# hridaybavle/semantic_slam

Measured on AMD Instinct MI355X. Metric: graph-optimize LM iters/sec (5k poses, 1k landmarks), higher is better.
Workload: dtype f64

## Files before the change

### include/sslam.h

```cpp
#ifndef SSLAM_H
#define SSLAM_H

#include <stdint.h>

#ifdef __cplusplus
extern "C" {
#endif

#define SSLAM_OK 0
#define SSLAM_ERR_INVALID (-1)
#define SSLAM_ERR_NO_DEVICE (-2)
#define SSLAM_ERR_HIP (-3)
#define SSLAM_ERR_NUMERIC (-4)
#define SSLAM_ERR_TOO_FEW_EDGES (-5)
#define SSLAM_ERR_UNSUPPORTED (-6)
#define SSLAM_ERR_IO (-7)

const char* sslam_last_error(void);
int sslam_device_count(void);
void* sslam_pinned_alloc(size_t bytes);
void sslam_pinned_free(void* p);

typedef struct sslam_graph sslam_graph;

// ... 68 lines not shown
sslam_batch* sslam_batch_create(sslam_graph* const* graphs, int n);
sslam_batch* sslam_batch_create_streams(sslam_graph* const* graphs, int n, int n_streams);
void sslam_batch_destroy(sslam_batch* b);
int sslam_batch_upload(sslam_batch* b);
int sslam_batch_download(sslam_batch* b);
int sslam_batch_optimize(sslam_batch* b, int max_iters, sslam_opt_stats* out );
int sslam_batch_marginals(sslam_batch* b, const int32_t* req, int n, double* out_blocks);
int sslam_comm_unique_id(char id_out[128]);
int sslam_batch_comm_init(sslam_batch* b, const char id_in[128], int rank, int world);
int sslam_batch_set_edge_shard(sslam_batch* b, int rank, int world);
int64_t sslam_batch_linearize_hb(sslam_batch* b, double* h_and_b, int64_t capacity);
int sslam_batch_time_linearize(sslam_batch* b, int repeats, double* ms_per_build);
int sslam_batch_time_solver(sslam_batch* b, int repeats, double* factor_ms, double* solve_ms);
int64_t sslam_batch_linearize_bytes(const sslam_batch* b);
int sslam_batch_info(sslam_batch* b, const char* key, double* value);
int sslam_batch_set_profiling(sslam_batch* b, int enable);
int sslam_batch_kernel_time(sslam_batch* b, const char* name, double* total_ms, int64_t* launches);

typedef struct sslam_seg sslam_seg;

typedef struct sslam_seg_params {
  double num_point_seg;
  double norm_point_thres;
  double planar_area;
  float max_depth_change_factor;
  float normal_smoothing_size;
  float angular_threshold;
  float distance_threshold;
  float maximum_curvature;
  int min_contour_points;
// ... 154 lines not shown
```

### semantic_slam_amd/_lib.py

```python
from __future__ import annotations

import ctypes as C
import os
import subprocess

_PKG = os.path.dirname(os.path.abspath(__file__))
_LIB = None


def library_path() -> str:
    return os.path.join(_PKG, "libsslam_hip.so")


def build_library(force: bool = False) -> str:
    args = ["make", "-C", os.path.join(_PKG, "csrc"), "-s"]
    if force:
        args.append("-B")
    subprocess.check_call(args)
    return library_path()


class OptStats(C.Structure):
    _fields_ = [("iterations", C.c_int), ("trials", C.c_int), ("status", C.c_int), ("host_plan_us", C.c_int),
                ("chi2_before", C.c_double), ("chi2_after", C.c_double), ("lambda_", C.c_double),
# ... 56 lines not shown
        "sslam_batch_create": (vp, [C.POINTER(vp), ci]),
        "sslam_batch_create_streams": (vp, [C.POINTER(vp), ci, ci]),
        "sslam_batch_destroy": (None, [vp]),
        "sslam_batch_upload": (ci, [vp]),
        "sslam_batch_download": (ci, [vp]),
        "sslam_batch_optimize": (ci, [vp, ci, C.POINTER(OptStats)]),
        "sslam_batch_marginals": (ci, [vp, C.POINTER(C.c_int32), ci, dp]),
        "sslam_comm_unique_id": (ci, [C.c_char_p]),
        "sslam_batch_comm_init": (ci, [vp, C.c_char_p, ci, ci]),
        "sslam_batch_set_edge_shard": (ci, [vp, ci, ci]),
        "sslam_batch_linearize_hb": (i64, [vp, dp, i64]),
        "sslam_batch_time_linearize": (ci, [vp, ci, dp]),
        "sslam_batch_time_solver": (ci, [vp, ci, dp, dp]),
        "sslam_batch_linearize_bytes": (i64, [vp]),
        "sslam_batch_info": (ci, [vp, C.c_char_p, dp]),
        "sslam_batch_set_profiling": (ci, [vp, ci]),
        "sslam_batch_kernel_time": (ci, [vp, C.c_char_p, dp, C.POINTER(i64)]),
    }
    for name, (res, args) in sig.items():
        fn = getattr(lib, name)
        fn.restype = res
        fn.argtypes = args
    _LIB = lib
    return lib
```

### semantic_slam_amd/csrc/chol_plan.hpp

```cpp
#pragma once
#include <algorithm>
#include <array>
#include <cstdint>
#include <cstdio>
#include <cstdlib>
#include <cstring>
#include <functional>
#include <map>
#include <queue>
#include <string>
#include <unordered_map>
#include <utility>
#include <vector>

namespace sslam {
#ifdef SSLAM_PLAN_TIMERS
#include <chrono>
#define SSLAM_PT_INIT auto pt_ = std::chrono::steady_clock::now();
#define SSLAM_PT(name) { auto n_ = std::chrono::steady_clock::now(); fprintf(stderr, "[plan-timer] %-14s %.3f ms\n", name, std::chrono::duration<double, std::milli>(n_ - pt_).count()); pt_ = n_; }
#else
#define SSLAM_PT_INIT
#define SSLAM_PT(name)
#endif

// ... 61 lines not shown
};
struct CholOpts {
  int cap_leaf = -1;
  int cap_tail = 4608;
  int max_blocks = 224;
  int tail_width = -1;
  int mid_width = -1;
  int cap_mid = 1800;
  int nt_mid = 128;
  int nt_ftail = 256;
  int pcap_mid = 16;
  int nt_bleaf = 0, nt_bmid = 0, nt_btail = 0;
  int nt_leaf = -1, nt_tail = 512;
  int min_chunk = 4;
  int split_min = 4096;
  int pcap_leaf = 4, pcap_tail = 32;
  int group_cap = -1;
  int group_blocks = 1024;
  int ustage = -1;
  int order = 1;
  double order_mul = -1;
  int order_add = -1;
  int order_bits_max = 2048;
  bool dump = false;
  int front = -1;
  int flow = 1;
  void from_env() {
    {
      static bool warned = false;
      if (!warned) {
// ... 10 lines not shown
    std::string str(e);
    size_t pos = 0;
    while (pos < str.size()) {
      size_t end = str.find(',', pos);
      if (end == std::string::npos) end = str.size();
      const std::string kv = str.substr(pos, end - pos);
      pos = end + 1;
      const size_t eq = kv.find('=');
      if (eq == std::string::npos) continue;
      const std::string k = kv.substr(0, eq), v = kv.substr(eq + 1);
      const int iv = atoi(v.c_str());
      if (k == "cap_leaf") cap_leaf = iv; else if (k == "cap_mid") cap_mid = iv; else if (k == "cap_tail") cap_tail = iv;
      else if (k == "max_blocks") max_blocks = iv; else if (k == "tail_width") tail_width = iv; else if (k == "mid_width") mid_width = iv;
      else if (k == "nt_leaf") { nt_leaf = iv; nt_leaf_set = true; } else if (k == "nt_mid") nt_mid = iv; else if (k == "nt_ftail") nt_ftail = iv; else if (k == "nt_bleaf") nt_bleaf = iv; else if (k == "nt_bmid") nt_bmid = iv; else if (k == "nt_btail") nt_btail = iv; else if (k == "nt_tail") nt_tail = iv;
      else if (k == "min_chunk") min_chunk = std::max(1, iv); else if (k == "split_min") split_min = std::max(2, iv);
      else if (k == "pcap_leaf") pcap_leaf = iv; else if (k == "pcap_mid") pcap_mid = iv; else if (k == "pcap_tail") pcap_tail = iv;
      else if (k == "group_cap") group_cap = iv; else if (k == "group_blocks") group_blocks = iv; else if (k == "ustage") ustage = iv;
      else if (k == "order_bits_max") order_bits_max = iv; else if (k == "flow") flow = iv; else if (k == "front") front = iv; else if (k == "dump") dump = iv != 0;
      else if (k == "order") order = (v == "mindeg" || v == "0") ? 0 : 1;
      else if (k == "order_mul") order_mul = atof(v.c_str()); else if (k == "order_add") order_add = iv;
      else fprintf(stderr, "[sslam] SSLAM_CHOL_OPTS: unknown key '%s'\n", k.c_str());
    }
  }
  bool nt_leaf_set = false;
};

inline bool chol_throughput_regime(int B, int block_rows) { return B >= 32 || (B >= 2 && block_rows >= 8000); }
inline bool chol_opts_normalise(CholOpts& opt, int B, int block_rows) {
  auto one_of = [](int v, std::initializer_list<int> set) { return std::find(set.begin(), set.end(), v) != set.end(); };
  if (opt.nt_tail != 1024) opt.nt_tail = 512;
  if (!one_of(opt.nt_leaf, {-1, 128, 256, 512, 1024})) opt.nt_leaf = 64;
  if (!one_of(opt.nt_mid, {256, 512})) opt.nt_mid = 128;
  if (opt.nt_tail == 1024) opt.nt_ftail = 1024;
  else if (!one_of(opt.nt_ftail, {128, 256, 1024})) opt.nt_ftail = 512;
  if (!one_of(opt.nt_btail, {128, 256})) opt.nt_btail = 512;
  for (int* nt : {&opt.nt_bleaf, &opt.nt_bmid})
    if (*nt <= 0) *nt = 0;
    else if (!one_of(*nt, {128, 256, 512, 1024})) *nt = 64;
  const bool want_flow = opt.flow != 0 && B < 8 && !chol_throughput_regime(B, block_rows) && opt.nt_tail == 512 && opt.group_cap <= 0 && !opt.nt_leaf_set;
  if (want_flow) { opt.nt_leaf = opt.nt_tail; opt.mid_width = 0; }
  return want_flow;
}

struct CholHost {
  int ncol = 0, nlevels = 0, dim = 0, B = 0, npiece = 0;
  int64_t lnz = 0;
  int64_t unz = 0;
  std::vector<ColMeta> col; std::vector<BlkMeta> blk; std::vector<UpdMeta> upd; std::vector<ItemMeta> item; std::vector<MbMeta> mb;
  std::vector<ILevel> ilv; std::vector<PieceMeta> piece;
  std::vector<AsmSrc> asrc, usrc; std::vector<FwdMeta> fwd; std::vector<UItem> uitem; std::vector<UMb> umb;
  std::vector<RCol> rcol; std::vector<UpdMeta> rupd;
  std::vector<int> lvl_ptr, lvl_cols;
  std::vector<int> plv_ptr, plv_pieces;
  std::vector<PieceMeta> lpiece;
  std::vector<int> tail_ptr, tail_pieces;
  std::vector<int> plv_lds_f, plv_lds_b;
  std::vector<int> plv_nt, plv_cls;
  int tail_lds_f = 0, tail_lds_b = 0;
  int nt_leaf = 64, nt_mid = 128, nt_tail = 512, nt_ftail = 256, nt_bleaf = 0, nt_bmid = 0, nt_btail = 0, ustage = 0;
  bool front = false;
  std::string front_why;
  std::vector<uint32_t> fblob;
  std::vector<FrontGrp> fgrp, lfgrp;
  std::vector<int> plv_lds_ff;
  int tail_lds_ff = 0;
  int64_t funz = 0;
  std::string error;
};

namespace chol_detail {

struct GraphSym {
// ... 800 lines not shown
    pm.nus = (int)out.usrc.size() - pm.us0;
  }
  out.unz = ucur;
  SSLAM_PT("piece loop")
  if (!right_ok) { out.rupd.clear(); out.rcol.assign(ncol, RCol{0, 0}); }
  auto lds_f = [&](int p) {
    const PieceMeta& pm = out.piece[p];
    const int ustage = (piece_cls[p] >= 1 || !opt.ustage) ? 0 : 4 * pm.nuit + 4 * pm.numb + ((pm.nuu + 1) & ~1) + pm.nus + 2;
    return 4 * pm.nilv + ((pm.lsize + 1) & ~1) + 2 * ((pm.ysize + 1) & ~1) + 4 * pm.nb + 3 * pm.nc + 2 * pm.nit_i + ((pm.nu_i + 1) & ~1) + 2 * pm.nimb + pm.nas + ustage +
           kItemDoubles * piece_pmax[p] + 8 + (piece_cls[p] >= 1 ? pm.nc + 2 : 0);
  };
  auto lds_b = [&](int p) {
    const PieceMeta& pm = out.piece[p];
    return 4 * pm.nilv + 36 * pm.nint + ((pm.ysize + 1) & ~1) + 7 * pm.nb + 3 * pm.nc + 12;
  };
  {
    std::vector<int> ptr{0}, launch_order, lnt, lcls;
    launch_order.reserve(out.plv_pieces.size());
    const int cut[3] = {640, 853, 1280};
    for (int l = 0; l < nplv; ++l) {
      std::vector<int> ps, pmid;
      for (int q = out.plv_ptr[l]; q < out.plv_ptr[l + 1]; ++q) (piece_cls[out.plv_pieces[q]] == 1 ? pmid : ps).push_back(out.plv_pieces[q]);
      const int n = (int)ps.size();
      if (n >= opt.split_min) {
        std::stable_sort(ps.begin(), ps.end(), [&](int a, int b) { return lds_b(a) < lds_b(b); });
        int q0 = 0;
        for (int k = 0; k < 3 && q0 < n; ++k) {
          int q1 = q0;
          while (q1 < n && lds_b(ps[q1]) <= cut[k]) ++q1;
          if (q1 - q0 >= opt.split_min / 2 && n - q1 >= opt.split_min / 2) { for (int q = q0; q < q1; ++q) launch_order.push_back(ps[q]); ptr.push_back((int)launch_order.size()); lnt.push_back(opt.nt_leaf); lcls.push_back(0); q0 = q1; }
        }
        for (int q = q0; q < n; ++q) launch_order.push_back(ps[q]);
      } else {
        for (int p : ps) launch_order.push_back(p);
      }
      if ((int)launch_order.size() > ptr.back()) { ptr.push_back((int)launch_order.size()); lnt.push_back(opt.nt_leaf); lcls.push_back(0); }
      if (!pmid.empty()) { for (int p : pmid) launch_order.push_back(p); ptr.push_back((int)launch_order.size()); lnt.push_back(opt.nt_mid); lcls.push_back(1); }
    }
    out.plv_nt = lnt; out.plv_cls = lcls;
    out.plv_pieces = launch_order;
    out.plv_ptr = ptr;
  }
  const int nlaunch = (int)out.plv_ptr.size() - 1;
  out.lpiece.clear();
  out.lpiece.reserve(npiece);
  for (int p : out.plv_pieces) out.lpiece.push_back(out.piece[p]);
  for (int p : out.tail_pieces) out.lpiece.push_back(out.piece[p]);
  out.plv_lds_f.assign(nlaunch, 0); out.plv_lds_b.assign(nlaunch, 0);
  for (int l = 0; l < nlaunch; ++l)
    for (int q = out.plv_ptr[l]; q < out.plv_ptr[l + 1]; ++q) {
      out.plv_lds_f[l] = std::max(out.plv_lds_f[l], lds_f(out.plv_pieces[q]));
      out.plv_lds_b[l] = std::max(out.plv_lds_b[l], lds_b(out.plv_pieces[q]));
    }
  for (int p : out.tail_pieces) { out.tail_lds_f = std::max(out.tail_lds_f, lds_f(p)); out.tail_lds_b = std::max(out.tail_lds_b, lds_b(p)); }
  if (opt.front > 0) {
    FrontHost F;
    front_build(FrontIn{ncol, npiece, ncomp, bp, brow, boff, bsrc, bfmt, col_comp, col_piece, col_dim, col_xoff, col_yoff, col_il, comp_parent, comp_R}, out.piece, out.ilv, F);
    for (int p = 0; p < npiece && F.ok; ++p) {
      const int nt = piece_tail[p] ? opt.nt_ftail : (piece_cls[p] == 1 ? opt.nt_mid : opt.nt_leaf);
      for (int l = 0; l < out.piece[p].nilv; ++l) {
        const ILevel& lv = out.ilv[out.piece[p].ilv0 + l];
        if (lv.c1 - lv.c0 > 2 * (nt / 8)) { F.ok = false; F.why = "a level of a piece has more columns than the workgroup's teams hold"; break; }
      }
    }
    out.front = F.ok; out.front_why = F.why;
    if (F.ok) {
      out.fblob.swap(F.blob); out.fgrp.swap(F.grp); out.funz = F.unz;
      out.lfgrp.reserve(npiece);
      for (int p : out.plv_pieces) out.lfgrp.push_back(out.fgrp[p]);
      for (int p : out.tail_pieces) out.lfgrp.push_back(out.fgrp[p]);
      out.plv_lds_ff.assign(nlaunch, 0);
      for (int l = 0; l < nlaunch; ++l)
        for (int q = out.plv_ptr[l]; q < out.plv_ptr[l + 1]; ++q) out.plv_lds_ff[l] = std::max(out.plv_lds_ff[l], F.lds[out.plv_pieces[q]]);
      for (int p : out.tail_pieces) out.tail_lds_ff = std::max(out.tail_lds_ff, F.lds[p]);
    }
    SSLAM_PT("front tables")
  }
  if (opt.dump) {
    fprintf(stderr, "[chol-dump] B %d cols %d blocks %d lnz %lld unz %lld updates %zu (internal items %zu, U items %zu) column-levels %d pieces %d piece-levels %d tail pieces %zu\n",
            B, ncol, nblk, (long long)lnz, (long long)out.unz, out.upd.size(), out.item.size(), out.uitem.size(), nlev, npiece, nplv, out.tail_pieces.size());
    for (int l = 0; l < nlaunch; ++l)
      fprintf(stderr, "[chol-dump]   launch %d: %d pieces x %d threads, LDS factor %d B backward %d B\n", l, out.plv_ptr[l + 1] - out.plv_ptr[l], out.plv_nt[l],
              out.plv_lds_f[l] * 8, out.plv_lds_b[l] * 8);
    int tmax = 0, tlv = 0;
    for (int g = 0; g < B; ++g) tmax = std::max(tmax, out.tail_ptr[g + 1] - out.tail_ptr[g]);
    for (int q = out.tail_ptr[0]; q < out.tail_ptr[std::min(1, B)]; ++q) tlv += out.piece[out.tail_pieces[q]].nilv;
    fprintf(stderr, "[chol-dump]   tail: <= %d pieces per graph (graph 0: %d internal levels), LDS factor %d B backward %d B\n", tmax, tlv,
            out.tail_lds_f * 8, out.tail_lds_b * 8);
  }
  return 0;
}

}
```

### semantic_slam_amd/csrc/graph_engine.hpp

```cpp
#pragma once
#include <hip/hip_runtime.h>
#include <algorithm>
#include <array>
#include <cstdint>
#include <cstring>
#include <map>
#include <string>
#include <vector>
#include "graph_host.hpp"
#include "graph_kernels.hpp"
#include "sslam_common.hpp"

namespace sslam {

struct CholPlan;
void chol_plan_free(CholPlan*);
void batch_comm_destroy(void* comm);

struct KernelTimer {
  double total_ms = 0;
  int64_t launches = 0;
};

struct DevArena {
// ... 177 lines not shown
      *out = (T*)p;
      return 0;
    }
    b.arena->note_direct(p, n * sizeof(T));
  } else { SSLAM_HIP_TRY(hipMalloc(&p, n * sizeof(T))); b.allocs.push_back(p); }
  if (zero) SSLAM_HIP_TRY(hipMemsetAsync(p, 0, n * sizeof(T), b.stream));
  *out = (T*)p;
  return 0;
}


struct SymIn;
void chol_sym_input(const Batch& b, SymIn& in);
int chol_plan_build(Batch& b);
int chol_plan_launches(const Batch& b);
int chol_factor_and_forward(Batch& b, bool flat = false);
int chol_backward(Batch& b);
int chol_set_active(Batch& b, const std::vector<char>* active);
int64_t chol_plan_lnz(const Batch& b);
int chol_plan_levels(const Batch& b);
bool chol_plan_front(const Batch& b);
bool chol_plan_flow(const Batch& b);
int chol_solve_flow(Batch& b);
int chol_lm_step_flow(Batch& b, int max_iters);
int chol_plan_lm_launches(const Batch& b, bool spec);
bool chol_plan_flow_rk(const Batch& b);
bool chol_plan_spec_rk(const Batch& b);
bool chol_plan_spec(const Batch& b);
int chol_spec_mode(const Batch& b);
int chol_lm_step_spec(Batch& b, int max_iters);
// ... 8 lines not shown
```

### semantic_slam_amd/csrc/sslam_chol.hip

```cpp
#include <hip/hip_runtime.h>
#include <algorithm>
#include <cstdio>
#include <cstring>
#include <mutex>
#include <type_traits>
#include <vector>

#include "../../include/sslam.h"
#include "graph_engine.hpp"
#include "chol_plan.hpp"

namespace sslam {

struct CholView {
  int ncol, nlevels, dim, npiece;
  const ColMeta* col;
  const BlkMeta* blk;
  const UpdMeta* upd;
  const ItemMeta* item;
  const MbMeta* mb;
  const ILevel* ilv;
  const PieceMeta* piece;
  const PieceMeta* lpiece;
  int ltail0;
// ... 22 lines not shown
  double *Lval = nullptr, *Uval = nullptr, *y = nullptr, *x = nullptr, *pose_trial = nullptr, *lmk_trial = nullptr, *part_e = nullptr, *part_a = nullptr;
  int *fail = nullptr, *flow = nullptr;
  int* err = nullptr;
  const double *pose_cur = nullptr, *lmk_cur = nullptr;
  long long sL = 0, sU = 0, sy = 0, sx = 0, spose = 0, slmk = 0, spe = 0, spa = 0, sflow = 0;
  int g0 = 0, g1 = 0;
  int after = 0;
  int* ctl = nullptr;
};

struct CholPlan {
  CholView C{};
  SpecLanes spec{};
  std::vector<int> plv_ptr, plv_lds_f, plv_lds_b, plv_nt, plv_cls;
  std::vector<int> plv_lds_ff;
  int tail_lds_ff = 0;
  bool front = false;
  int tail_lds_f = 0, tail_lds_b = 0, tail_total = 0, nt_tail = 512, nt_ftail = 256, nt_bleaf = 0, nt_bmid = 0, nt_btail = 0, ustage = 0;
  std::vector<void*> allocs;
  DevArena* arena = nullptr;
  int64_t lnz = 0, unz = 0;
  std::vector<int> lp_graph;
  std::vector<int> c_ptr;
  int* d_idx = nullptr;
  size_t idx_cap = 0;
  bool compact = false;
  bool flow = false;
  int flow_grid = 0;
  int spec_grid = 0;
  double flow_need = 1.0, spec_need = 1.0;
  bool rk_flow_ok = false, rk_spec_ok = false;
  bool flow_narrow = false;
  int flow_epoch = 0;
  int lm_epoch = 0;
  int spec_epoch = 0;
  int2* d_dep = nullptr;
  int* d_flow = nullptr;
  std::vector<int> h_cparent;
// ... 1347 lines not shown
  if (b.chol) { chol_plan_free(b.chol); b.chol = nullptr; }
  SSLAM_HIP_TRY(hipSetDevice(b.device));
  SymIn in;
  chol_sym_input(b, in);
  CholOpts opt;
  opt.from_env();
  const int flow_mode = opt.flow;
  const bool want_flow = chol_opts_normalise(opt, b.V.B, b.V.nPr + b.V.nLr);
  CholHost H;
  if (chol_symbolic(in, opt, H)) return set_error(SSLAM_ERR_NUMERIC, "Cholesky plan: %s", H.error.c_str());
  CholPlan* P = new CholPlan();
  b.chol = P;
  P->arena = b.arena;
  CholView& C = P->C;
  C.ncol = H.ncol; C.nlevels = H.nlevels; C.dim = H.dim; C.npiece = H.npiece;
  P->plv_ptr = H.plv_ptr; P->plv_lds_f = H.plv_lds_f; P->plv_lds_b = H.plv_lds_b; P->plv_nt = H.plv_nt; P->plv_cls = H.plv_cls;
  P->tail_lds_f = H.tail_lds_f; P->tail_lds_b = H.tail_lds_b; P->tail_total = (int)H.tail_pieces.size(); P->nt_tail = H.nt_tail; P->nt_ftail = H.nt_ftail; P->nt_bleaf = H.nt_bleaf; P->nt_bmid = H.nt_bmid; P->nt_btail = H.nt_btail; P->ustage = H.ustage;
  P->lnz = H.lnz;
  {
    std::vector<int> yoff_col(H.dim + 1, -1);
    for (int j = 0; j < H.ncol; ++j) yoff_col[H.col[j].yoff] = j;
    P->h_cparent.assign(H.ncol, -1);
    P->h_xoff_col.assign(H.dim + 1, -1);
    for (int j = 0; j < H.ncol; ++j) {
      if (H.col[j].nb > 1) P->h_cparent[j] = yoff_col[H.blk[H.col[j].b0 + 1].yoff_row];
      P->h_xoff_col[H.col[j].xoff] = j;
    }
  }
  int rc;
  if ((rc = up_to_dev(*P, b.stream, H.col, &C.col))) return rc;
// ... 328 lines not shown
  if (!stage) stage = &local;
  SSLAM_HIP_TRY(hipMemcpyAsync(stage, d_err, sizeof(int), hipMemcpyDeviceToHost, b.stream));
  SSLAM_HIP_TRY(hipStreamSynchronize(b.stream));
  if (*stage) {
    SSLAM_HIP_TRY(hipMemsetAsync(d_err, 0, sizeof(int), b.stream));
    SSLAM_HIP_TRY(hipStreamSynchronize(b.stream));
    return set_error(SSLAM_ERR_HIP, "sparse Cholesky: a dependency wait of the single-launch factorisation timed out (the graphs concerned carry a failed trial)");
  }
  return 0;
}

int64_t chol_plan_lnz(const Batch& b) { return b.chol ? b.chol->lnz : 0; }
int chol_plan_levels(const Batch& b) { return b.chol ? b.chol->C.nlevels : 0; }
bool chol_plan_front(const Batch& b) { return b.chol && b.chol->front; }
int chol_plan_launches(const Batch& b) { return b.chol ? (int)b.chol->plv_lds_f.size() + (b.chol->tail_total > 0 ? 1 : 0) : 0; }

int chol_set_active(Batch& b, const std::vector<char>* active) {
  if (!b.chol) return 0;
  CholPlan& P = *b.chol;
  P.compact = false;
  if (!active) return 0;
  const int B = b.V.B;
  int na = 0;
  for (int g = 0; g < B; ++g) na += (*active)[g] ? 1 : 0;
  if (B < 8 || na == 0 || 2 * na > B) return 0;
  const int nplv = (int)P.plv_lds_f.size();
  std::vector<int> idx;
  idx.reserve(P.lp_graph.size() * (size_t)na / B + 64);
  P.c_ptr.assign(nplv + 2, 0);
  for (int l = 0; l < nplv; ++l) {
    P.c_ptr[l] = (int)idx.size();
    for (int q = P.plv_ptr[l]; q < P.plv_ptr[l + 1]; ++q) if ((*active)[P.lp_graph[q]]) idx.push_back(q);
  }
  P.c_ptr[nplv] = (int)idx.size();
  if (P.tail_total > 0) for (int g = 0; g < B; ++g) if ((*active)[g]) idx.push_back(g);
  P.c_ptr[nplv + 1] = (int)idx.size();
  if (idx.size() > P.idx_cap) {
    if (P.d_idx) (void)hipFree(P.d_idx);
    P.d_idx = nullptr; P.idx_cap = 0;
    SSLAM_HIP_TRY(hipMalloc((void**)&P.d_idx, (idx.size() + 1024) * sizeof(int)));
    P.idx_cap = idx.size() + 1024;
  }
  if (!idx.empty()) SSLAM_HIP_TRY(hipMemcpyAsync(P.d_idx, idx.data(), idx.size() * sizeof(int), hipMemcpyHostToDevice, b.stream));
  SSLAM_HIP_TRY(hipStreamSynchronize(b.stream));
  P.compact = true;
  return 0;
}

int chol_factor_and_forward(Batch& b, bool flat) {
  CholPlan& P = *b.chol;
  P.C.flat_L = flat ? 1 : 0;
// ... 51 lines not shown
int chol_backward(Batch& b) {
  CholPlan& P = *b.chol;
  const CholView& C = P.C;
  if (C.flat_L) return set_error(SSLAM_ERR_INVALID, "chol_backward needs the class-interleaved factor (the last factorisation was a flat one)");
  ScopedTimer t(b, "solve");
  const int nplv = (int)P.plv_lds_b.size();
  const int ntail = P.compact ? P.c_ptr[nplv + 1] - P.c_ptr[nplv] : b.V.B;
  if (P.tail_total > 0 && ntail > 0) {
    const int* idx = P.compact ? P.d_idx + P.c_ptr[nplv] : nullptr;
    const int rc = with_width(BackTailWidths{}, P.nt_btail, [&](auto w) {
      hipLaunchKernelGGL(k_chol_back_tail<decltype(w)::value>, dim3(ntail), dim3(w), (size_t)P.tail_lds_b * sizeof(double), b.stream, C, (const double*)C.y, b.V.x,
                         (const LmState*)b.V.lm, idx);
    });
    if (rc) return rc;
  }
  for (int l = nplv - 1; l >= 0; --l) {
    const int n = P.compact ? P.c_ptr[l + 1] - P.c_ptr[l] : P.plv_ptr[l + 1] - P.plv_ptr[l];
    if (n <= 0) continue;
    const int* idx = P.compact ? P.d_idx + P.c_ptr[l] : nullptr;
    const int ovr = P.plv_cls[l] == 1 ? P.nt_bmid : P.nt_bleaf;
    const int rc = with_width(LeafWidths{}, ovr > 0 ? ovr : P.plv_nt[l], [&](auto w) {
      hipLaunchKernelGGL(k_chol_back_pieces<decltype(w)::value>, dim3(n), dim3(w), (size_t)P.plv_lds_b[l] * sizeof(double), b.stream, C, P.plv_ptr[l],
                         (const double*)C.y, b.V.x, (const LmState*)b.V.lm, idx);
    });
    if (rc) return rc;
  }
  hipError_t e = hipGetLastError();
  if (e != hipSuccess) return set_error(SSLAM_ERR_HIP, "cholesky solve launch: %s", hipGetErrorString(e));
  return 0;
}

int chol_marginal_blocks(Batch& b, const std::vector<MarginalReq>& reqs, double* out) {
  CholPlan& P = *b.chol;
  const CholView& C = P.C;
  const size_t n = reqs.size();
  if (n == 0) return 0;
  if (!C.flat_L) return set_error(SSLAM_ERR_INVALID, "chol_marginal_blocks needs the flat factor (chol_factor_and_forward(b, true))");
// ... 83 lines not shown
```

### semantic_slam_amd/csrc/sslam_graph.hip

```cpp
#include <hip/hip_runtime.h>
#include <rccl/rccl.h>
#include <dlfcn.h>
#include <algorithm>
#include <chrono>
#include <cmath>
#include <cstdio>
#include <cstring>
#include <map>
#include <memory>
#include <string>
#include <unordered_map>
#include <thread>
#include <vector>

#include "../../include/sslam.h"
#include "graph_host.hpp"
#include "graph_kernels.hpp"
#include "sslam_common.hpp"
#include "graph_engine.hpp"
#include "chol_plan.hpp"

namespace sslam {


// ... 2572 lines not shown
    if (kk == "streams") { *value = (double)h->parts.size(); return 0; }
    double acc = 0;
    for (sslam_batch* p : h->parts) {
      double v = 0;
      const int rc = sslam_batch_info(p, key, &v);
      if (rc) return rc;
      acc = kk == "factor_levels" ? std::max(acc, v) : acc + v;
    }
    *value = acc;
    return 0;
  }
  if (std::string(key) == "streams") { *value = 1; return 0; }
  Batch& b = h->b;
  const std::string k(key);
  int rc;
  if ((k == "factor_lnz" || k == "factor_levels" || k == "factor_launches" || k == "factor_front" || k == "factor_bytes") && !b.chol && (rc = chol_plan_build(b))) return rc;
  const double dim = 6.0 * b.V.nPr + 3.0 * b.V.nLr;
  if (k == "factor_lnz") *value = (double)chol_plan_lnz(b);
  else if (k == "factor_levels") *value = (double)chol_plan_levels(b);
  else if (k == "factor_launches") *value = (double)chol_plan_launches(b);
  else if (k == "factor_front") *value = chol_plan_front(b) ? 1.0 : 0.0;
  else if (k == "h_doubles") *value = (double)b.V.h_total;
  else if (k == "dim") *value = dim;
  else if (k == "allreduce_calls") *value = (double)b.allreduce_calls;
  else if (k == "lm_fused_launches") *value = (double)chol_plan_lm_launches(b, false);
  else if (k == "lm_spec_rounds") *value = (double)chol_plan_lm_launches(b, true);
  else if (k == "factor_bytes") *value = 8.0 * ((double)b.V.h_total + dim + (double)chol_plan_lnz(b) + dim);
  else return set_error(SSLAM_ERR_INVALID, "unknown info key '%s'", key);
  return 0;
}
int sslam_batch_set_profiling(sslam_batch* h, int enable) {
  if (!h) return set_error(SSLAM_ERR_INVALID, "null batch");
  for (sslam_batch* p : h->parts) sslam_batch_set_profiling(p, enable);
  h->b.profiling = enable != 0;
  h->b.timers.clear();
  return 0;
}
int sslam_batch_kernel_time(sslam_batch* h, const char* name, double* total_ms, int64_t* launches) {
  if (!h || !name) return set_error(SSLAM_ERR_INVALID, "null argument");
  if (!h->parts.empty()) {
    double t = 0; int64_t n = 0;
    for (sslam_batch* p : h->parts) { double a = 0; int64_t c = 0; sslam_batch_kernel_time(p, name, &a, &c); t += a; n += c; }
    if (total_ms) *total_ms = t;
    if (launches) *launches = n;
// ... 33 lines not shown
int64_t sslam_debug_plan_array(void* p, const char* name, void* out, int64_t cap_bytes) {
  if (!p || !name) return set_error(SSLAM_ERR_INVALID, "null argument");
  const CholHost& H = ((sslam_debug_plan*)p)->H;
  const std::string k(name);
  const void* src = nullptr; int64_t bytes = 0;
  const sslam_debug_plan& DP = *(sslam_debug_plan*)p;
  int scal[17] = {H.ncol, H.nlevels, H.dim, H.B, H.npiece, (int)H.lnz, H.tail_lds_f, H.tail_lds_b, H.nt_leaf, H.nt_tail, (int)DP.h_total,
                  DP.sc[11], DP.sc[12], DP.sc[13], DP.sc[14], DP.sc[15], (int)H.unz};
#define ARR(nm, vec) if (k == nm) { src = (vec).data(); bytes = (int64_t)(vec).size() * sizeof((vec)[0]); }
  ARR("col", H.col) ARR("blk", H.blk) ARR("upd", H.upd) ARR("item", H.item) ARR("mb", H.mb) ARR("ilv", H.ilv) ARR("piece", H.piece)
  ARR("lvl_ptr", H.lvl_ptr) ARR("lvl_cols", H.lvl_cols) ARR("plv_ptr", H.plv_ptr) ARR("plv_pieces", H.plv_pieces)
  ARR("ppoff", DP.ppoff) ARR("plblk", DP.plblk) ARR("tail_ptr", H.tail_ptr)
  ARR("asrc", H.asrc) ARR("usrc", H.usrc) ARR("fwd", H.fwd) ARR("uitem", H.uitem) ARR("umb", H.umb) ARR("tail_pieces", H.tail_pieces) ARR("plv_lds_f", H.plv_lds_f) ARR("plv_lds_b", H.plv_lds_b)
  ARR("rcol", H.rcol) ARR("rupd", H.rupd) ARR("plv_nt", H.plv_nt) ARR("plv_cls", H.plv_cls)
  ARR("fblob", H.fblob) ARR("fgrp", H.fgrp) ARR("plv_lds_ff", H.plv_lds_ff)
#undef ARR
  int fscal[4] = {H.front ? 1 : 0, (int)H.funz, H.tail_lds_ff, 0};
  if (k == "fscalars") { src = fscal; bytes = sizeof fscal; }
  if (k == "scalars") { src = scal; bytes = sizeof scal; }
  static const char* known[] = {"col", "blk", "upd", "item", "mb", "ilv", "piece", "lvl_ptr", "lvl_cols", "plv_ptr", "plv_pieces", "ppoff", "plblk",
                                "tail_ptr", "tail_pieces", "plv_lds_f", "plv_lds_b", "scalars", "asrc", "usrc", "fwd", "uitem", "umb", "rcol", "rupd", "plv_nt", "plv_cls",
                                "fblob", "fgrp", "plv_lds_ff", "fscalars"};
  bool ok = false;
  for (const char* q : known) ok |= (k == q);
  if (!ok) return set_error(SSLAM_ERR_INVALID, "unknown plan array '%s'", name);
  if (out && cap_bytes >= bytes && bytes > 0) memcpy(out, src, (size_t)bytes);
  return bytes;
}

}
```

### semantic_slam_amd/graph_slam.py

```python
from __future__ import annotations

import ctypes as C
from typing import Sequence

import numpy as np

from ._lib import load_library, OptStats

ERR_TOO_FEW_EDGES = -5


class SslamError(RuntimeError):
    def __init__(self, code: int, msg: str):
        super().__init__(f"sslam error {code}: {msg}")
        self.code = code


def _dptr(a: np.ndarray):
    return a.ctypes.data_as(C.POINTER(C.c_double))


def _check(lib, rc: int) -> int:
    if rc < 0:
        raise SslamError(rc, lib.sslam_last_error().decode())
# ... 335 lines not shown
        return ms.value

    def time_solver(self, repeats: int = 5):
        f = C.c_double(0); s = C.c_double(0)
        _check(self._lib, self._lib.sslam_batch_time_solver(self._h, repeats, C.byref(f), C.byref(s)))
        return f.value, s.value

    def linearize_bytes(self) -> int:
        return int(self._lib.sslam_batch_linearize_bytes(self._h))

    def info(self, key: str) -> float:
        v = C.c_double(0)
        _check(self._lib, self._lib.sslam_batch_info(self._h, key.encode(), C.byref(v)))
        return v.value

    def set_profiling(self, on: bool):
        _check(self._lib, self._lib.sslam_batch_set_profiling(self._h, 1 if on else 0))

    def kernel_time(self, name: str):
        ms = C.c_double(0); n = C.c_int64(0)
        _check(self._lib, self._lib.sslam_batch_kernel_time(self._h, name.encode(), C.byref(ms), C.byref(n)))
        return ms.value, n.value
```

Measured before the change: 34790.

## Split Cholesky piece launches by LDS residency class and decouple backward launches

The supernodal Cholesky plan now sorts the pieces of each level by how many workgroups per CU their LDS need allows, and cuts launches where that residency class changes, so small pieces are no longer held to the occupancy of the largest piece in the launch. The backward solve gets its own launch partition (blv_ptr) with per-launch LDS sizing, independent of the factor launches. The old size-cut scheme is kept only for the single-launch flow mode. This costs extra kernel launches and extra host-side planning, and it adds a debug query that compares planned residency against what the HIP occupancy API reports.

```diff
diff --git a/include/sslam.h b/include/sslam.h
--- a/include/sslam.h
+++ b/include/sslam.h
@@ -106,6 +106,7 @@
 int sslam_batch_time_solver(sslam_batch* b, int repeats, double* factor_ms, double* solve_ms);
 int64_t sslam_batch_linearize_bytes(const sslam_batch* b);
 int sslam_batch_info(sslam_batch* b, const char* key, double* value);
+int sslam_debug_launch_residency(sslam_batch* b, int backward, int launch, int* planned, int* runtime);
 int sslam_batch_set_profiling(sslam_batch* b, int enable);
 int sslam_batch_kernel_time(sslam_batch* b, const char* name, double* total_ms, int64_t* launches);
 
diff --git a/semantic_slam_amd/_lib.py b/semantic_slam_amd/_lib.py
--- a/semantic_slam_amd/_lib.py
+++ b/semantic_slam_amd/_lib.py
@@ -94,6 +94,7 @@
         "sslam_batch_time_solver": (ci, [vp, ci, dp, dp]),
         "sslam_batch_linearize_bytes": (i64, [vp]),
         "sslam_batch_info": (ci, [vp, C.c_char_p, dp]),
+        "sslam_debug_launch_residency": (ci, [vp, ci, ci, C.POINTER(ci), C.POINTER(ci)]),
         "sslam_batch_set_profiling": (ci, [vp, ci]),
         "sslam_batch_kernel_time": (ci, [vp, C.c_char_p, dp, C.POINTER(i64)]),
     }
diff --git a/semantic_slam_amd/csrc/chol_plan.hpp b/semantic_slam_amd/csrc/chol_plan.hpp
--- a/semantic_slam_amd/csrc/chol_plan.hpp
+++ b/semantic_slam_amd/csrc/chol_plan.hpp
@@ -99,6 +99,11 @@
   int nt_leaf = -1, nt_tail = 512;
   int min_chunk = 4;
   int split_min = 4096;
+  int lds_budget = 160 * 1024;
+  int lds_granule = 8;
+  int res_front = -1, res_back = -1;
+  int lds_cut = 1;
+  bool single_launch = false;
   int pcap_leaf = 4, pcap_tail = 32;
   int group_cap = -1;
   int group_blocks = 1024;
@@ -139,6 +144,8 @@
       else if (k == "max_blocks") max_blocks = iv; else if (k == "tail_width") tail_width = iv; else if (k == "mid_width") mid_width = iv;
       else if (k == "nt_leaf") { nt_leaf = iv; nt_leaf_set = true; } else if (k == "nt_mid") nt_mid = iv; else if (k == "nt_ftail") nt_ftail = iv; else if (k == "nt_bleaf") nt_bleaf = iv; else if (k == "nt_bmid") nt_bmid = iv; else if (k == "nt_btail") nt_btail = iv; else if (k == "nt_tail") nt_tail = iv;
       else if (k == "min_chunk") min_chunk = std::max(1, iv); else if (k == "split_min") split_min = std::max(2, iv);
+      else if (k == "lds_budget") lds_budget = std::max(1024, iv); else if (k == "lds_granule") lds_granule = std::max(8, iv);
+      else if (k == "res_front") res_front = iv; else if (k == "res_back") res_back = iv; else if (k == "lds_cut") lds_cut = iv;
       else if (k == "pcap_leaf") pcap_leaf = iv; else if (k == "pcap_mid") pcap_mid = iv; else if (k == "pcap_tail") pcap_tail = iv;
       else if (k == "group_cap") group_cap = iv; else if (k == "group_blocks") group_blocks = iv; else if (k == "ustage") ustage = iv;
       else if (k == "order_bits_max") order_bits_max = iv; else if (k == "flow") flow = iv; else if (k == "front") front = iv; else if (k == "dump") dump = iv != 0;
@@ -150,6 +157,13 @@
   bool nt_leaf_set = false;
 };
 
+constexpr int kFrontWavesPerSimd = 3, kRecordWavesPerSimd = 4, kBackWavesPerSimd = 6, kBackWavesPerSimd64 = 8;
+inline int chol_residency_cap(int waves_per_simd, int nt) { return std::max(1, std::min(nt > 64 ? 16 : 32, 4 * waves_per_simd * 64 / std::max(nt, 64))); }
+inline int chol_residency(const CholOpts& opt, int need_bytes, int cap) {
+  const int g = std::max(opt.lds_granule, 1);
+  const int alloc = std::max(g, (need_bytes + g - 1) / g * g);
+  return std::max(1, std::min(cap, opt.lds_budget / alloc));
+}
 inline bool chol_throughput_regime(int B, int block_rows) { return B >= 32 || (B >= 2 && block_rows >= 8000); }
 inline bool chol_opts_normalise(CholOpts& opt, int B, int block_rows) {
   auto one_of = [](int v, std::initializer_list<int> set) { return std::find(set.begin(), set.end(), v) != set.end(); };
@@ -164,6 +178,7 @@
     else if (!one_of(*nt, {128, 256, 512, 1024})) *nt = 64;
   const bool want_flow = opt.flow != 0 && B < 8 && !chol_throughput_regime(B, block_rows) && opt.nt_tail == 512 && opt.group_cap <= 0 && !opt.nt_leaf_set;
   if (want_flow) { opt.nt_leaf = opt.nt_tail; opt.mid_width = 0; }
+  opt.single_launch = want_flow;
   return want_flow;
 }
 
@@ -181,6 +196,9 @@
   std::vector<int> tail_ptr, tail_pieces;
   std::vector<int> plv_lds_f, plv_lds_b;
   std::vector<int> plv_nt, plv_cls;
+  std::vector<int> blv_ptr, blv_launch, blv_lds_b;
+  std::vector<int> plv_res, blv_res;
+  std::vector<int> piece_lds_f, piece_lds_b;
   int tail_lds_f = 0, tail_lds_b = 0;
   int nt_leaf = 64, nt_mid = 128, nt_tail = 512, nt_ftail = 256, nt_bleaf = 0, nt_bmid = 0, nt_btail = 0, ustage = 0;
   bool front = false;
@@ -1011,34 +1029,81 @@
     const PieceMeta& pm = out.piece[p];
     return 4 * pm.nilv + 36 * pm.nint + ((pm.ysize + 1) & ~1) + 7 * pm.nb + 3 * pm.nc + 12;
   };
+  FrontHost F;
+  if (opt.front > 0) {
+    front_build(FrontIn{ncol, npiece, ncomp, bp, brow, boff, bsrc, bfmt, col_comp, col_piece, col_dim, col_xoff, col_yoff, col_il, comp_parent, comp_R}, out.piece, out.ilv, F);
+    for (int p = 0; p < npiece && F.ok; ++p) {
+      const int nt = piece_tail[p] ? opt.nt_ftail : (piece_cls[p] == 1 ? opt.nt_mid : opt.nt_leaf);
+      for (int l = 0; l < out.piece[p].nilv; ++l) {
+        const ILevel& lv = out.ilv[out.piece[p].ilv0 + l];
+        if (lv.c1 - lv.c0 > 2 * (nt / 8)) { F.ok = false; F.why = "a level of a piece has more columns than the workgroup's teams hold"; break; }
+      }
+    }
+    out.front = F.ok; out.front_why = F.why;
+    if (F.ok) { out.fblob.swap(F.blob); out.fgrp.swap(F.grp); out.funz = F.unz; }
+    SSLAM_PT("front tables")
+  }
+  auto need_f = [&](int p) { return out.front ? F.lds[p] : lds_f(p); };
+  const int nt_back_leaf = opt.nt_bleaf > 0 ? opt.nt_bleaf : opt.nt_leaf, nt_back_mid = opt.nt_bmid > 0 ? opt.nt_bmid : opt.nt_mid;
+  auto cap_f = [&](int nt) { return opt.res_front > 0 ? opt.res_front : chol_residency_cap(out.front ? kFrontWavesPerSimd : kRecordWavesPerSimd, nt); };
+  auto cap_b = [&](int nt) { return opt.res_back > 0 ? opt.res_back : chol_residency_cap(nt <= 64 ? kBackWavesPerSimd64 : kBackWavesPerSimd, nt); };
+  auto res_f = [&](int p) { return chol_residency(opt, 8 * need_f(p), cap_f(opt.nt_leaf)); };
+  auto res_b = [&](int p) { return chol_residency(opt, 8 * lds_b(p), cap_b(nt_back_leaf)); };
   {
-    std::vector<int> ptr{0}, launch_order, lnt, lcls;
+    std::vector<int> ptr{0}, launch_order, lnt, lcls, bptr{0}, blaunch;
     launch_order.reserve(out.plv_pieces.size());
     const int cut[3] = {640, 853, 1280};
+    const int part_min = opt.split_min / 2;
+    auto cut_classes = [&](const std::vector<int>& ps, int q0, int q1, auto&& cls, auto&& emit) {
+      int a = q0;
+      for (int q = q0 + 1; q < q1; ++q)
+        if (cls(ps[q]) != cls(ps[q - 1]) && q - a >= part_min && q1 - q >= part_min) { emit(a, q); a = q; }
+      emit(a, q1);
+    };
     for (int l = 0; l < nplv; ++l) {
       std::vector<int> ps, pmid;
       for (int q = out.plv_ptr[l]; q < out.plv_ptr[l + 1]; ++q) (piece_cls[out.plv_pieces[q]] == 1 ? pmid : ps).push_back(out.plv_pieces[q]);
       const int n = (int)ps.size();
-      if (n >= opt.split_min) {
-        std::stable_sort(ps.begin(), ps.end(), [&](int a, int b) { return lds_b(a) < lds_b(b); });
-        int q0 = 0;
-        for (int k = 0; k < 3 && q0 < n; ++k) {
-          int q1 = q0;
-          while (q1 < n && lds_b(ps[q1]) <= cut[k]) ++q1;
-          if (q1 - q0 >= opt.split_min / 2 && n - q1 >= opt.split_min / 2) { for (int q = q0; q < q1; ++q) launch_order.push_back(ps[q]); ptr.push_back((int)launch_order.size()); lnt.push_back(opt.nt_leaf); lcls.push_back(0); q0 = q1; }
+      if (opt.single_launch) {
+        if (n >= opt.split_min) {
+          std::stable_sort(ps.begin(), ps.end(), [&](int a, int b) { return lds_b(a) < lds_b(b); });
+          int q0 = 0;
+          for (int k = 0; k < 3 && q0 < n; ++k) {
+            int q1 = q0;
+            while (q1 < n && lds_b(ps[q1]) <= cut[k]) ++q1;
+            if (q1 - q0 >= part_min && n - q1 >= part_min) { for (int q = q0; q < q1; ++q) launch_order.push_back(ps[q]); ptr.push_back((int)launch_order.size()); lnt.push_back(opt.nt_leaf); lcls.push_back(0); q0 = q1; }
+          }
+          for (int q = q0; q < n; ++q) launch_order.push_back(ps[q]);
+        } else {
+          for (int p : ps) launch_order.push_back(p);
         }
-        for (int q = q0; q < n; ++q) launch_order.push_back(ps[q]);
-      } else {
+        if ((int)launch_order.size() > ptr.back()) { ptr.push_back((int)launch_order.size()); lnt.push_back(opt.nt_leaf); lcls.push_back(0); }
+        for (size_t k = bptr.size(); k < ptr.size(); ++k) { bptr.push_back(ptr[k]); blaunch.push_back((int)k - 1); }
+      } else if (n > 0) {
+        const bool cutting = opt.lds_cut != 0 && n >= opt.split_min;
+        const int base = (int)launch_order.size();
+        if (cutting) std::stable_sort(ps.begin(), ps.end(), [&](int a, int b) { return res_f(a) > res_f(b); });
+        auto factor_launch = [&](int q0, int q1) {
+          if (cutting) std::stable_sort(ps.begin() + q0, ps.begin() + q1, [&](int a, int b) { return res_b(a) > res_b(b); });
+          auto back_launch = [&](int a, int b) { bptr.push_back(base + b); blaunch.push_back((int)lnt.size()); };
+          if (cutting) cut_classes(ps, q0, q1, res_b, back_launch); else back_launch(q0, q1);
+          ptr.push_back(base + q1); lnt.push_back(opt.nt_leaf); lcls.push_back(0);
+        };
+        if (cutting) cut_classes(ps, 0, n, res_f, factor_launch); else factor_launch(0, n);
         for (int p : ps) launch_order.push_back(p);
       }
-      if ((int)launch_order.size() > ptr.back()) { ptr.push_back((int)launch_order.size()); lnt.push_back(opt.nt_leaf); lcls.push_back(0); }
-      if (!pmid.empty()) { for (int p : pmid) launch_order.push_back(p); ptr.push_back((int)launch_order.size()); lnt.push_back(opt.nt_mid); lcls.push_back(1); }
+      if (!pmid.empty()) {
+        for (int p : pmid) launch_order.push_back(p);
+        bptr.push_back((int)launch_order.size()); blaunch.push_back((int)lnt.size());
+        ptr.push_back((int)launch_order.size()); lnt.push_back(opt.nt_mid); lcls.push_back(1);
+      }
     }
     out.plv_nt = lnt; out.plv_cls = lcls;
     out.plv_pieces = launch_order;
     out.plv_ptr = ptr;
-  }
-  const int nlaunch = (int)out.plv_ptr.size() - 1;
+    out.blv_ptr = bptr; out.blv_launch = blaunch;
+  }
+  const int nlaunch = (int)out.plv_ptr.size() - 1, nblaunch = (int)out.blv_ptr.size() - 1;
   out.lpiece.clear();
   out.lpiece.reserve(npiece);
   for (int p : out.plv_pieces) out.lpiece.push_back(out.piece[p]);
@@ -1049,36 +1114,35 @@
       out.plv_lds_f[l] = std::max(out.plv_lds_f[l], lds_f(out.plv_pieces[q]));
       out.plv_lds_b[l] = std::max(out.plv_lds_b[l], lds_b(out.plv_pieces[q]));
     }
+  out.blv_lds_b.assign(nblaunch, 0);
+  for (int k = 0; k < nblaunch; ++k)
+    for (int q = out.blv_ptr[k]; q < out.blv_ptr[k + 1]; ++q) out.blv_lds_b[k] = std::max(out.blv_lds_b[k], lds_b(out.plv_pieces[q]));
   for (int p : out.tail_pieces) { out.tail_lds_f = std::max(out.tail_lds_f, lds_f(p)); out.tail_lds_b = std::max(out.tail_lds_b, lds_b(p)); }
-  if (opt.front > 0) {
-    FrontHost F;
-    front_build(FrontIn{ncol, npiece, ncomp, bp, brow, boff, bsrc, bfmt, col_comp, col_piece, col_dim, col_xoff, col_yoff, col_il, comp_parent, comp_R}, out.piece, out.ilv, F);
-    for (int p = 0; p < npiece && F.ok; ++p) {
-      const int nt = piece_tail[p] ? opt.nt_ftail : (piece_cls[p] == 1 ? opt.nt_mid : opt.nt_leaf);
-      for (int l = 0; l < out.piece[p].nilv; ++l) {
-        const ILevel& lv = out.ilv[out.piece[p].ilv0 + l];
-        if (lv.c1 - lv.c0 > 2 * (nt / 8)) { F.ok = false; F.why = "a level of a piece has more columns than the workgroup's teams hold"; break; }
-      }
-    }
-    out.front = F.ok; out.front_why = F.why;
-    if (F.ok) {
-      out.fblob.swap(F.blob); out.fgrp.swap(F.grp); out.funz = F.unz;
-      out.lfgrp.reserve(npiece);
-      for (int p : out.plv_pieces) out.lfgrp.push_back(out.fgrp[p]);
-      for (int p : out.tail_pieces) out.lfgrp.push_back(out.fgrp[p]);
-      out.plv_lds_ff.assign(nlaunch, 0);
-      for (int l = 0; l < nlaunch; ++l)
-        for (int q = out.plv_ptr[l]; q < out.plv_ptr[l + 1]; ++q) out.plv_lds_ff[l] = std::max(out.plv_lds_ff[l], F.lds[out.plv_pieces[q]]);
-      for (int p : out.tail_pieces) out.tail_lds_ff = std::max(out.tail_lds_ff, F.lds[p]);
-    }
-    SSLAM_PT("front tables")
-  }
+  if (out.front) {
+    out.lfgrp.reserve(npiece);
+    for (int p : out.plv_pieces) out.lfgrp.push_back(out.fgrp[p]);
+    for (int p : out.tail_pieces) out.lfgrp.push_back(out.fgrp[p]);
+    out.plv_lds_ff.assign(nlaunch, 0);
+    for (int l = 0; l < nlaunch; ++l)
+      for (int q = out.plv_ptr[l]; q < out.plv_ptr[l + 1]; ++q) out.plv_lds_ff[l] = std::max(out.plv_lds_ff[l], F.lds[out.plv_pieces[q]]);
+    for (int p : out.tail_pieces) out.tail_lds_ff = std::max(out.tail_lds_ff, F.lds[p]);
+  }
+  out.piece_lds_f.resize(npiece); out.piece_lds_b.resize(npiece);
+  for (int p = 0; p < npiece; ++p) { out.piece_lds_f[p] = need_f(p); out.piece_lds_b[p] = lds_b(p); }
+  out.plv_res.assign(nlaunch, 0); out.blv_res.assign(nblaunch, 0);
+  for (int l = 0; l < nlaunch; ++l)
+    out.plv_res[l] = chol_residency(opt, 8 * (out.front ? out.plv_lds_ff[l] : out.plv_lds_f[l]), cap_f(out.plv_nt[l]));
+  for (int k = 0; k < nblaunch; ++k)
+    out.blv_res[k] = chol_residency(opt, 8 * out.blv_lds_b[k], cap_b(out.plv_cls[out.blv_launch[k]] == 1 ? nt_back_mid : nt_back_leaf));
   if (opt.dump) {
     fprintf(stderr, "[chol-dump] B %d cols %d blocks %d lnz %lld unz %lld updates %zu (internal items %zu, U items %zu) column-levels %d pieces %d piece-levels %d tail pieces %zu\n",
             B, ncol, nblk, (long long)lnz, (long long)out.unz, out.upd.size(), out.item.size(), out.uitem.size(), nlev, npiece, nplv, out.tail_pieces.size());
     for (int l = 0; l < nlaunch; ++l)
-      fprintf(stderr, "[chol-dump]   launch %d: %d pieces x %d threads, LDS factor %d B backward %d B\n", l, out.plv_ptr[l + 1] - out.plv_ptr[l], out.plv_nt[l],
-              out.plv_lds_f[l] * 8, out.plv_lds_b[l] * 8);
+      fprintf(stderr, "[chol-dump]   launch %d: %d pieces x %d threads, LDS factor %d B (%d per CU) backward %d B\n", l, out.plv_ptr[l + 1] - out.plv_ptr[l], out.plv_nt[l],
+              (out.front ? out.plv_lds_ff[l] : out.plv_lds_f[l]) * 8, out.plv_res[l], out.plv_lds_b[l] * 8);
+    for (int k = 0; k < nblaunch; ++k)
+      fprintf(stderr, "[chol-dump]   backward launch %d (in launch %d): %d pieces, LDS %d B (%d per CU)\n", k, out.blv_launch[k], out.blv_ptr[k + 1] - out.blv_ptr[k],
+              out.blv_lds_b[k] * 8, out.blv_res[k]);
     int tmax = 0, tlv = 0;
     for (int g = 0; g < B; ++g) tmax = std::max(tmax, out.tail_ptr[g + 1] - out.tail_ptr[g]);
     for (int q = out.tail_ptr[0]; q < out.tail_ptr[std::min(1, B)]; ++q) tlv += out.piece[out.tail_pieces[q]].nilv;
diff --git a/semantic_slam_amd/csrc/graph_engine.hpp b/semantic_slam_amd/csrc/graph_engine.hpp
--- a/semantic_slam_amd/csrc/graph_engine.hpp
+++ b/semantic_slam_amd/csrc/graph_engine.hpp
@@ -215,6 +215,8 @@
 void chol_sym_input(const Batch& b, SymIn& in);
 int chol_plan_build(Batch& b);
 int chol_plan_launches(const Batch& b);
+int chol_plan_back_launches(const Batch& b);
+int chol_plan_launch_residency(const Batch& b, bool backward, int l, int* planned, int* runtime);
 int chol_factor_and_forward(Batch& b, bool flat = false);
 int chol_backward(Batch& b);
 int chol_set_active(Batch& b, const std::vector<char>* active);
diff --git a/semantic_slam_amd/csrc/sslam_chol.hip b/semantic_slam_amd/csrc/sslam_chol.hip
--- a/semantic_slam_amd/csrc/sslam_chol.hip
+++ b/semantic_slam_amd/csrc/sslam_chol.hip
@@ -60,6 +60,7 @@
   SpecLanes spec{};
   std::vector<int> plv_ptr, plv_lds_f, plv_lds_b, plv_nt, plv_cls;
   std::vector<int> plv_lds_ff;
+  std::vector<int> blv_ptr, blv_launch, blv_lds_b, plv_res, blv_res;
   int tail_lds_ff = 0;
   bool front = false;
   int tail_lds_f = 0, tail_lds_b = 0, tail_total = 0, nt_tail = 512, nt_ftail = 256, nt_bleaf = 0, nt_bmid = 0, nt_btail = 0, ustage = 0;
@@ -68,6 +69,7 @@
   int64_t lnz = 0, unz = 0;
   std::vector<int> lp_graph;
   std::vector<int> c_ptr;
+  std::vector<int> cb_ptr;
   int* d_idx = nullptr;
   size_t idx_cap = 0;
   bool compact = false;
@@ -1445,6 +1447,7 @@
   P->arena = b.arena;
   CholView& C = P->C;
   C.ncol = H.ncol; C.nlevels = H.nlevels; C.dim = H.dim; C.npiece = H.npiece;
+  P->blv_ptr = H.blv_ptr; P->blv_launch = H.blv_launch; P->blv_lds_b = H.blv_lds_b; P->plv_res = H.plv_res; P->blv_res = H.blv_res;
   P->plv_ptr = H.plv_ptr; P->plv_lds_f = H.plv_lds_f; P->plv_lds_b = H.plv_lds_b; P->plv_nt = H.plv_nt; P->plv_cls = H.plv_cls;
   P->tail_lds_f = H.tail_lds_f; P->tail_lds_b = H.tail_lds_b; P->tail_total = (int)H.tail_pieces.size(); P->nt_tail = H.nt_tail; P->nt_ftail = H.nt_ftail; P->nt_bleaf = H.nt_bleaf; P->nt_bmid = H.nt_bmid; P->nt_btail = H.nt_btail; P->ustage = H.ustage;
   P->lnz = H.lnz;
@@ -1803,6 +1806,47 @@
 int chol_plan_levels(const Batch& b) { return b.chol ? b.chol->C.nlevels : 0; }
 bool chol_plan_front(const Batch& b) { return b.chol && b.chol->front; }
 int chol_plan_launches(const Batch& b) { return b.chol ? (int)b.chol->plv_lds_f.size() + (b.chol->tail_total > 0 ? 1 : 0) : 0; }
+int chol_plan_back_launches(const Batch& b) { return b.chol ? (int)b.chol->blv_lds_b.size() + (b.chol->tail_total > 0 ? 1 : 0) : 0; }
+int chol_plan_launch_residency(const Batch& b, bool backward, int l, int* planned, int* runtime) {
+  if (!b.chol) return set_error(SSLAM_ERR_INVALID, "no Cholesky plan");
+  const CholPlan& P = *b.chol;
+  const int n = backward ? (int)P.blv_lds_b.size() : (int)P.plv_lds_f.size();
+  if (l < 0 || l >= n) return set_error(SSLAM_ERR_INVALID, "launch %d of %d", l, n);
+  const int fl = backward ? P.blv_launch[l] : l;
+  const bool mid = P.plv_cls[fl] == 1;
+  const void* fn = nullptr;
+  int nt = P.plv_nt[fl];
+  size_t lds;
+  if (backward) {
+    const int ovr = mid ? P.nt_bmid : P.nt_bleaf;
+    if (ovr > 0) nt = ovr;
+    lds = (size_t)P.blv_lds_b[l] * sizeof(double);
+    const int rc = with_width(LeafWidths{}, nt, [&](auto w) { fn = (const void*)k_chol_back_pieces<decltype(w)::value>; });
+    if (rc) return rc;
+  } else if (P.front) {
+    lds = (size_t)P.plv_lds_ff[l] * sizeof(double);
+    const int rc = with_width(LeafWidths{}, nt, [&](auto w) {
+      constexpr int NT = decltype(w)::value;
+      fn = mid ? (const void*)k_front_pieces<NT, true> : (const void*)k_front_pieces<NT, false>;
+    });
+    if (rc) return rc;
+  } else {
+    lds = (size_t)P.plv_lds_f[l] * sizeof(double);
+    const int rc = mid ? with_width(MidWidths{}, nt, [&](auto w) {
+      constexpr int NT = decltype(w)::value;
+      fn = P.C.rupd ? (const void*)k_chol_pieces<NT, false, true> : (const void*)k_chol_pieces<NT, false, false>;
+    }) : with_width(LeafWidths{}, nt, [&](auto w) {
+      constexpr int NT = decltype(w)::value;
+      fn = P.ustage ? (const void*)k_chol_pieces<NT, true> : (const void*)k_chol_pieces<NT, false>;
+    });
+    if (rc) return rc;
+  }
+  int per_cu = 0;
+  SSLAM_HIP_TRY(hipOccupancyMaxActiveBlocksPerMultiprocessor(&per_cu, fn, nt, lds));
+  if (planned) *planned = backward ? P.blv_res[l] : P.plv_res[l];
+  if (runtime) *runtime = per_cu;
+  return 0;
+}
 
 int chol_set_active(Batch& b, const std::vector<char>* active) {
   if (!b.chol) return 0;
@@ -1824,6 +1868,15 @@
   P.c_ptr[nplv] = (int)idx.size();
   if (P.tail_total > 0) for (int g = 0; g < B; ++g) if ((*active)[g]) idx.push_back(g);
   P.c_ptr[nplv + 1] = (int)idx.size();
+  {
+    const int nblv = (int)P.blv_lds_b.size();
+    P.cb_ptr.assign(nblv + 1, P.c_ptr[nplv]);
+    int at = 0;
+    for (int k = 0; k < nblv; ++k) {
+      P.cb_ptr[k] = at;
+      while (at < P.c_ptr[nplv] && idx[at] < P.blv_ptr[k + 1]) ++at;
+    }
+  }
   if (idx.size() > P.idx_cap) {
     if (P.d_idx) (void)hipFree(P.d_idx);
     P.d_idx = nullptr; P.idx_cap = 0;
@@ -1905,13 +1958,14 @@
     });
     if (rc) return rc;
   }
-  for (int l = nplv - 1; l >= 0; --l) {
-    const int n = P.compact ? P.c_ptr[l + 1] - P.c_ptr[l] : P.plv_ptr[l + 1] - P.plv_ptr[l];
+  for (int k = (int)P.blv_lds_b.size() - 1; k >= 0; --k) {
+    const int n = P.compact ? P.cb_ptr[k + 1] - P.cb_ptr[k] : P.blv_ptr[k + 1] - P.blv_ptr[k];
     if (n <= 0) continue;
-    const int* idx = P.compact ? P.d_idx + P.c_ptr[l] : nullptr;
+    const int* idx = P.compact ? P.d_idx + P.cb_ptr[k] : nullptr;
+    const int l = P.blv_launch[k];
     const int ovr = P.plv_cls[l] == 1 ? P.nt_bmid : P.nt_bleaf;
     const int rc = with_width(LeafWidths{}, ovr > 0 ? ovr : P.plv_nt[l], [&](auto w) {
-      hipLaunchKernelGGL(k_chol_back_pieces<decltype(w)::value>, dim3(n), dim3(w), (size_t)P.plv_lds_b[l] * sizeof(double), b.stream, C, P.plv_ptr[l],
+      hipLaunchKernelGGL(k_chol_back_pieces<decltype(w)::value>, dim3(n), dim3(w), (size_t)P.blv_lds_b[k] * sizeof(double), b.stream, C, P.blv_ptr[k],
                          (const double*)C.y, b.V.x, (const LmState*)b.V.lm, idx);
     });
     if (rc) return rc;
diff --git a/semantic_slam_amd/csrc/sslam_graph.hip b/semantic_slam_amd/csrc/sslam_graph.hip
--- a/semantic_slam_amd/csrc/sslam_graph.hip
+++ b/semantic_slam_amd/csrc/sslam_graph.hip
@@ -2610,11 +2610,12 @@
   Batch& b = h->b;
   const std::string k(key);
   int rc;
-  if ((k == "factor_lnz" || k == "factor_levels" || k == "factor_launches" || k == "factor_front" || k == "factor_bytes") && !b.chol && (rc = chol_plan_build(b))) return rc;
+  if ((k == "factor_lnz" || k == "factor_levels" || k == "factor_launches" || k == "solve_launches" || k == "factor_front" || k == "factor_bytes") && !b.chol && (rc = chol_plan_build(b))) return rc;
   const double dim = 6.0 * b.V.nPr + 3.0 * b.V.nLr;
   if (k == "factor_lnz") *value = (double)chol_plan_lnz(b);
   else if (k == "factor_levels") *value = (double)chol_plan_levels(b);
   else if (k == "factor_launches") *value = (double)chol_plan_launches(b);
+  else if (k == "solve_launches") *value = (double)chol_plan_back_launches(b);
   else if (k == "factor_front") *value = chol_plan_front(b) ? 1.0 : 0.0;
   else if (k == "h_doubles") *value = (double)b.V.h_total;
   else if (k == "dim") *value = dim;
@@ -2624,6 +2625,14 @@
   else if (k == "factor_bytes") *value = 8.0 * ((double)b.V.h_total + dim + (double)chol_plan_lnz(b) + dim);
   else return set_error(SSLAM_ERR_INVALID, "unknown info key '%s'", key);
   return 0;
+}
+int sslam_debug_launch_residency(sslam_batch* h, int backward, int launch, int* planned, int* runtime) {
+  if (!h) return set_error(SSLAM_ERR_INVALID, "null batch");
+  if (!h->parts.empty()) return set_error(SSLAM_ERR_UNSUPPORTED, "launch residency of a stream group: ask a plain batch");
+  Batch& b = h->b;
+  int rc;
+  if (!b.chol && (rc = chol_plan_build(b))) return rc;
+  return chol_plan_launch_residency(b, backward != 0, launch, planned, runtime);
 }
 int sslam_batch_set_profiling(sslam_batch* h, int enable) {
   if (!h) return set_error(SSLAM_ERR_INVALID, "null batch");
@@ -2687,13 +2696,15 @@
   ARR("asrc", H.asrc) ARR("usrc", H.usrc) ARR("fwd", H.fwd) ARR("uitem", H.uitem) ARR("umb", H.umb) ARR("tail_pieces", H.tail_pieces) ARR("plv_lds_f", H.plv_lds_f) ARR("plv_lds_b", H.plv_lds_b)
   ARR("rcol", H.rcol) ARR("rupd", H.rupd) ARR("plv_nt", H.plv_nt) ARR("plv_cls", H.plv_cls)
   ARR("fblob", H.fblob) ARR("fgrp", H.fgrp) ARR("plv_lds_ff", H.plv_lds_ff)
+  ARR("blv_ptr", H.blv_ptr) ARR("blv_launch", H.blv_launch) ARR("blv_lds_b", H.blv_lds_b) ARR("plv_res", H.plv_res) ARR("blv_res", H.blv_res)
+  ARR("piece_lds_f", H.piece_lds_f) ARR("piece_lds_b", H.piece_lds_b)
 #undef ARR
   int fscal[4] = {H.front ? 1 : 0, (int)H.funz, H.tail_lds_ff, 0};
   if (k == "fscalars") { src = fscal; bytes = sizeof fscal; }
   if (k == "scalars") { src = scal; bytes = sizeof scal; }
   static const char* known[] = {"col", "blk", "upd", "item", "mb", "ilv", "piece", "lvl_ptr", "lvl_cols", "plv_ptr", "plv_pieces", "ppoff", "plblk",
                                 "tail_ptr", "tail_pieces", "plv_lds_f", "plv_lds_b", "scalars", "asrc", "usrc", "fwd", "uitem", "umb", "rcol", "rupd", "plv_nt", "plv_cls",
-                                "fblob", "fgrp", "plv_lds_ff", "fscalars"};
+                                "fblob", "fgrp", "plv_lds_ff", "fscalars", "blv_ptr", "blv_launch", "blv_lds_b", "plv_res", "blv_res", "piece_lds_f", "piece_lds_b"};
   bool ok = false;
   for (const char* q : known) ok |= (k == q);
   if (!ok) return set_error(SSLAM_ERR_INVALID, "unknown plan array '%s'", name);
diff --git a/semantic_slam_amd/graph_slam.py b/semantic_slam_amd/graph_slam.py
--- a/semantic_slam_amd/graph_slam.py
+++ b/semantic_slam_amd/graph_slam.py
@@ -373,6 +373,11 @@
         _check(self._lib, self._lib.sslam_batch_info(self._h, key.encode(), C.byref(v)))
         return v.value
 
+    def launch_residency(self, backward: bool, launch: int):
+        a, b = C.c_int(0), C.c_int(0)
+        _check(self._lib, self._lib.sslam_debug_launch_residency(self._h, 1 if backward else 0, int(launch), C.byref(a), C.byref(b)))
+        return a.value, b.value
+
     def set_profiling(self, on: bool):
         _check(self._lib, self._lib.sslam_batch_set_profiling(self._h, 1 if on else 0))
 
```

New measurement: 33990. 0.977x the previous value.
